# IamJasonBian/Splendor-RL-Gym

Measured on NVIDIA B200. Metric: expanded states/sec (gen+dedup+score+top-k), higher is better.
Workload: dtype u64 keys / f64 scores

## Files before the change

### splendor-rl-gym_b200/csrc/spl_m2.cuh

```cuda
#pragma once
#include "spl_kernels.cuh"

namespace spl {

constexpr int GEM_STATES = 2898;
constexpr int NODE_BM_WORDS = 46;
constexpr int NODE_WORDS = 48;
constexpr uint64_t NODE_OCC = 1ull << 63;
constexpr int SMALL_ITEMS = 32;
constexpr int SMALL_W = 128;
constexpr int SM_TBL = 256;
constexpr int SM_STAGE = 48;
struct GroupArgs;
constexpr int NUM_CLS = 8;
constexpr int CLS_WARP = 6, CLS_CTA = 7;
constexpr int M2_WARPS = TILE / 32;
constexpr int BIG_DONE = 16;
constexpr int BIG_AT_BITS = 24;

__device__ __host__ __forceinline__ void mask_words(uint64_t lo, uint64_t hi, uint64_t &m0, uint64_t &m1) {
    m0 = (lo >> 15) | (hi << 49);
    m1 = (hi & HI_KEY_MASK) >> 15;
}
__device__ __host__ __forceinline__ uint64_t mask_hash(uint64_t m0, uint64_t m1) { return hash_key(m0, m1); }
// ... 181 lines not shown
#pragma unroll
    for (int q = 0; q < SORT_ITEMS; ++q) {
        const int64_t i = wbase + q * 32 + lane;
        const bool ok = i < n;
        v[q] = ok ? v_in[i] : 0;
        const uint32_t d = (uint32_t)(v[q] >> shift) & (SORT_BINS - 1);
        const unsigned act = __ballot_sync(0xffffffffu, ok);
        off[q] = 0;
        if (ok) {
            const unsigned peers = __match_any_sync(act, d);
            const int leader = __ffs(peers) - 1;
            uint32_t old = 0;
            if ((int)lane == leader) {
                old = whist[w][d];
                whist[w][d] = old + __popc(peers);
            }
            old = __shfl_sync(peers, old, leader);
            off[q] = (uint16_t)(old + __popc(peers & ((1u << lane) - 1)));
        }
        __syncwarp();
    }
    __syncthreads();
    {
        const uint32_t d = threadIdx.x;
        uint32_t run = 0;
        for (int ww = 0; ww < TILE / 32; ++ww) {
            const uint32_t c = whist[ww][d];
            whist[ww][d] = run;
            run += c;
        }
        uint32_t tot;
        const uint32_t ex = block_excl_scan(run, warp_sums, tot);
        dbase[d] = ex;
        gbase[d] = matrix_scanned[(uint64_t)d * ntiles + blockIdx.x];
        for (int ww = 0; ww < TILE / 32; ++ww) whist[ww][d] += ex;
    }
    __syncthreads();
#pragma unroll
    for (int q = 0; q < SORT_ITEMS; ++q) {
        const int64_t i = wbase + q * 32 + lane;
        if (i < n) stage[whist[w][(uint32_t)(v[q] >> shift) & (SORT_BINS - 1)] + off[q]] = v[q];
    }
    __syncthreads();
    const uint32_t cnt = (uint32_t)min((int64_t)SORT_TILE, n - tbase);
    for (uint32_t i = threadIdx.x; i < cnt; i += TILE) {
        const uint64_t x = stage[i];
        const uint32_t d = (uint32_t)(x >> shift) & (SORT_BINS - 1);
        v_out[gbase[d] + (i - dbase[d])] = x;
    }
}

constexpr int ITEM_KEY_LO = 34;
constexpr int OS_BITS = 10, OS_BINS = 1 << OS_BITS, OS_MAX_PASSES = 7;
constexpr int OS_DPT = OS_BINS / TILE;
static_assert(OS_DPT == 4, "the one-sweep pass moves the four digits of a thread as one 16-byte word");
constexpr int64_t OS_MAX_ITEMS = 1ll << 30;

__global__ void __launch_bounds__(TILE) os_hist_kernel(const uint64_t *__restrict__ v, int64_t n, int lo_bit, int passes,
                                                       uint32_t *__restrict__ hist) {
    extern __shared__ uint32_t os_sh[];
    for (int i = threadIdx.x; i < passes * OS_BINS; i += TILE) os_sh[i] = 0;
    __syncthreads();
    for (int64_t i = (int64_t)blockIdx.x * TILE + threadIdx.x; i < n; i += (int64_t)gridDim.x * TILE) {
        const uint64_t x = v[i] >> lo_bit;
        for (int p = 0; p < passes; ++p) atomicAdd(&os_sh[p * OS_BINS + ((uint32_t)(x >> (p * OS_BITS)) & (OS_BINS - 1))], 1u);
    }
    __syncthreads();
    for (int i = threadIdx.x; i < passes * OS_BINS; i += TILE) {
        const uint32_t c = os_sh[i];
        if (c) atomicAdd(hist + i, c);
    }
}
__global__ void __launch_bounds__(OS_BINS) os_base_kernel(uint32_t *hist) {
    __shared__ uint32_t ws[OS_BINS / 32];
    uint32_t *h = hist + blockIdx.x * OS_BINS;
    const unsigned lane = threadIdx.x & 31, w = threadIdx.x >> 5;
    const uint32_t c = h[threadIdx.x];
    const uint32_t inc = warp_incl_scan(c);
    if (lane == 31) ws[w] = inc;
    __syncthreads();
    if (w == 0) {
        const uint32_t x = ws[lane], xi = warp_incl_scan(x);
        ws[lane] = xi - x;
    }
    __syncthreads();
    h[threadIdx.x] = inc - c + ws[w];
}

struct OsSmem {
    uint64_t stage[SORT_TILE];
    uint32_t gbase[OS_BINS];
    uint16_t whist[TILE / 32][OS_BINS];
    uint16_t dbase[OS_BINS];
    uint32_t warp_sums[TILE / 32 + 1];
    uint32_t tile;
    uint32_t stage_p[SORT_TILE];
};
template <bool PAIR>
__global__ void __launch_bounds__(TILE, PAIR ? 3 : 4) os_scatter_kernel(const uint64_t *__restrict__ v_in, const uint32_t *__restrict__ p_in,
                                                                        int64_t n, int shift, const uint32_t *__restrict__ base ,
                                                                        uint32_t *status, Counters *ctr, int ticket_id,
                                                                        uint64_t *__restrict__ v_out, uint32_t *__restrict__ p_out) {
    extern __shared__ __align__(16) unsigned char smem_raw[];
    OsSmem &S = *reinterpret_cast<OsSmem *>(smem_raw);
    const unsigned lane = threadIdx.x & 31, w = threadIdx.x >> 5;
    if (threadIdx.x == 0) S.tile = atomicAdd(&ctr->ticket[ticket_id], 1u);
    for (int i = threadIdx.x; i < (TILE / 32) * OS_BINS / 2; i += TILE) reinterpret_cast<uint32_t *>(&S.whist[0][0])[i] = 0;
    __syncthreads();
    const uint32_t tile = S.tile;
    const int64_t tbase = (int64_t)tile * SORT_TILE, wbase = tbase + (int64_t)w * (32 * SORT_ITEMS);
    uint64_t v[SORT_ITEMS];
    uint32_t pl[PAIR ? SORT_ITEMS : 1];
    uint16_t off[SORT_ITEMS];
#pragma unroll
    for (int q = 0; q < SORT_ITEMS; ++q) {
        const int64_t i = wbase + q * 32 + lane;
        v[q] = i < n ? v_in[i] : 0;
        if (PAIR) pl[q] = i < n ? p_in[i] : 0;
    }
#pragma unroll
    for (int q = 0; q < SORT_ITEMS; ++q) {
        const bool ok = wbase + q * 32 + lane < n;
        const uint32_t d = (uint32_t)(v[q] >> shift) & (OS_BINS - 1);
        const unsigned act = __ballot_sync(0xffffffffu, ok);
        off[q] = 0;
        if (ok) {
            const unsigned peers = __match_any_sync(act, d);
            const int leader = __ffs(peers) - 1;
            uint32_t old = 0;
            if ((int)lane == leader) {
                old = S.whist[w][d];
                S.whist[w][d] = (uint16_t)(old + __popc(peers));
            }
            old = __shfl_sync(peers, old, leader);
            off[q] = (uint16_t)(old + __popc(peers & ((1u << lane) - 1)));
        }
        __syncwarp();
    }
    __syncthreads();
    const uint32_t d0 = threadIdx.x * OS_DPT;
    uint32_t cnt[OS_DPT] = {0, 0, 0, 0};
    for (int ww = 0; ww < TILE / 32; ++ww) {
        uint2 x = *reinterpret_cast<uint2 *>(&S.whist[ww][d0]);
        const uint32_t c0 = x.x & 0xffffu, c1 = x.x >> 16, c2 = x.y & 0xffffu, c3 = x.y >> 16;
        x.x = cnt[0] | (cnt[1] << 16); x.y = cnt[2] | (cnt[3] << 16);
        *reinterpret_cast<uint2 *>(&S.whist[ww][d0]) = x;
        cnt[0] += c0; cnt[1] += c1; cnt[2] += c2; cnt[3] += c3;
    }
    constexpr uint32_t VAL = (1u << 30) - 1;
    uint32_t *mine = status + (uint64_t)tile * OS_BINS + d0;
    {
        const uint32_t f = tile == 0 ? 2u << 30 : 1u << 30;
        uint4 a{f | cnt[0], f | cnt[1], f | cnt[2], f | cnt[3]};
        asm volatile("st.volatile.global.v4.u32 [%0], {%1, %2, %3, %4};" ::"l"(mine), "r"(a.x), "r"(a.y), "r"(a.z), "r"(a.w) : "memory");
    }
    {
        uint32_t tot;
        const uint32_t ex = block_excl_scan(cnt[0] + cnt[1] + cnt[2] + cnt[3], S.warp_sums, tot);
        const uint32_t e0 = ex, e1 = e0 + cnt[0], e2 = e1 + cnt[1], e3 = e2 + cnt[2];
        *reinterpret_cast<uint2 *>(&S.dbase[d0]) = uint2{e0 | (e1 << 16), e2 | (e3 << 16)};
        for (int ww = 0; ww < TILE / 32; ++ww) {
            uint2 x = *reinterpret_cast<uint2 *>(&S.whist[ww][d0]);
            x.x += e0 | (e1 << 16); x.y += e2 | (e3 << 16);
            *reinterpret_cast<uint2 *>(&S.whist[ww][d0]) = x;
        }
    }
    __syncthreads();
#pragma unroll
    for (int q = 0; q < SORT_ITEMS; ++q) {
        if (wbase + q * 32 + lane < n) {
            const uint32_t at = S.whist[w][(uint32_t)(v[q] >> shift) & (OS_BINS - 1)] + off[q];
            S.stage[at] = v[q];
            if (PAIR) S.stage_p[at] = pl[q];
        }
    }
    uint32_t ex[OS_DPT] = {0, 0, 0, 0};
    if (tile > 0) {
        unsigned open = 15;
        for (int64_t p = (int64_t)tile - 1; open; --p) {
            const uint32_t *src = status + (uint64_t)p * OS_BINS + d0;
            uint32_t s[OS_DPT];
            bool ready;
            do {
                asm volatile("ld.volatile.global.v4.u32 {%0, %1, %2, %3}, [%4];" : "=r"(s[0]), "=r"(s[1]), "=r"(s[2]), "=r"(s[3]) : "l"(src) : "memory");
                ready = true;
#pragma unroll
                for (int k = 0; k < OS_DPT; ++k) ready = ready && (!((open >> k) & 1) || (s[k] >> 30) != 0);
            } while (!ready);
#pragma unroll
            for (int k = 0; k < OS_DPT; ++k)
                if ((open >> k) & 1) {
                    ex[k] += s[k] & VAL;
                    if ((s[k] >> 30) == 2) open &= ~(1u << k);
                }
        }
        const uint32_t f = 2u << 30;
        asm volatile("st.volatile.global.v4.u32 [%0], {%1, %2, %3, %4};" ::"l"(mine), "r"(f | (ex[0] + cnt[0])), "r"(f | (ex[1] + cnt[1])),
                     "r"(f | (ex[2] + cnt[2])), "r"(f | (ex[3] + cnt[3])) : "memory");
    }
    {
        const uint4 b = *reinterpret_cast<const uint4 *>(base + d0);
        *reinterpret_cast<uint4 *>(&S.gbase[d0]) = uint4{b.x + ex[0], b.y + ex[1], b.z + ex[2], b.w + ex[3]};
    }
    __syncthreads();
    const uint32_t cnt_tile = (uint32_t)min((int64_t)SORT_TILE, n - tbase);
    for (uint32_t i = threadIdx.x; i < cnt_tile; i += TILE) {
        const uint64_t x = S.stage[i];
        const uint32_t d = (uint32_t)(x >> shift) & (OS_BINS - 1);
        const uint32_t to = S.gbase[d] + (i - S.dbase[d]);
        v_out[to] = x;
        if (PAIR) p_out[to] = S.stage_p[i];
    }
}

constexpr int RUN_ITEMS = 8;
__global__ void __launch_bounds__(TILE) m2_runs_kernel(const uint64_t *__restrict__ iv, int64_t n_items, uint32_t np,
                                                       const uint8_t *__restrict__ ntk8,
                                                       uint32_t *__restrict__ run_start, uint32_t *__restrict__ run_wpre,
                                                       uint64_t *status_f, uint64_t *status_w, Counters *ctr, int ticket_id) {
    __shared__ uint32_t warp_sums[TILE / 32 + 1];
    __shared__ uint32_t s_tile;
    __shared__ uint64_t s_fbase, s_wbase;
    if (threadIdx.x == 0) s_tile = atomicAdd(&ctr->ticket[ticket_id], 1u);
    __syncthreads();
    const uint32_t tile = s_tile;
    const int64_t b0 = ((int64_t)tile * TILE + threadIdx.x) * RUN_ITEMS;
    uint32_t flags = 0, w[RUN_ITEMS], fsum = 0, wsum = 0;
    uint64_t prev = (b0 > 0 && b0 - 1 < n_items) ? iv[b0 - 1] >> ITEM_KEY_LO : 0;
#pragma unroll
    for (int q = 0; q < RUN_ITEMS; ++q) {
        const int64_t i = b0 + q;
        w[q] = 0;
        if (i < n_items) {
            const uint64_t v = iv[i], k = v >> ITEM_KEY_LO;
            if (i == 0 || k != prev) { flags |= 1u << q; ++fsum; }
            prev = k;
            const uint32_t id = (uint32_t)v;
            w[q] = id < np ? ntk8[id] : 1u;
            wsum += w[q];
        }
    }
    uint32_t tot;
    const uint32_t ex = block_excl_scan(wsum << 12 | fsum, warp_sums, tot);
    if (threadIdx.x < 32) {
        const uint64_t e = lookback_exclusive(status_f, tile, tot & 0xfffu, 0);
        if (threadIdx.x == 0) s_fbase = e;
    } else if (threadIdx.x < 64) {
        const uint64_t e = lookback_exclusive(status_w, tile, tot >> 12, 0);
        if (threadIdx.x == 32) s_wbase = e;
    }
    __syncthreads();
    uint64_t r = s_fbase + (ex & 0xfffu), wp = s_wbase + (ex >> 12);
#pragma unroll
    for (int q = 0; q < RUN_ITEMS; ++q) {
        if (flags >> q & 1) {
            run_start[r] = (uint32_t)(b0 + q);
            run_wpre[r] = (uint32_t)wp;
            ++r;
        }
        wp += w[q];
    }
    if (b0 <= n_items - 1 && n_items - 1 < b0 + RUN_ITEMS) {
        run_start[r] = (uint32_t)n_items;
        run_wpre[r] = (uint32_t)wp;
// ... 604 lines not shown
```

### splendor-rl-gym_b200/csrc/splendor_b200.cu

```cuda
#include "../../include/splendor_b200.h"

#include <stdarg.h>
#include <stdio.h>
#include <string.h>

#include <algorithm>
#include <string>
#include <vector>

#include "spl_kernels.cuh"
#include "spl_m2.cuh"
#include "spl_shard.cuh"
#include "spl_realistic.cuh"
#include "spl_tables.cuh"

using namespace spl;

static std::string g_create_error;

struct DevBuf {
    void *p = nullptr;
    size_t cap = 0;
    ~DevBuf() { release(); }
    void release() {
// ... 184 lines not shown
            int r_ = fail(nullptr, e2_ == cudaErrorMemoryAllocation ? SPL_E_NOMEM : SPL_E_CUDA, "%s: %s", #call, \
                          cudaGetErrorString(e2_));                                                           \
            delete c;                                                                                         \
            return r_;                                                                                        \
        }                                                                                                     \
    } while (0)
    CKC(cudaSetDevice(c->device));
    size_t free_b = 0, total_b = 0;
    CKC(cudaMemGetInfo(&free_b, &total_b));
    c->max_table_bytes = cfg->max_table_bytes ? cfg->max_table_bytes : (uint64_t)(free_b * 0.6);
    c->chunk_user = cfg->chunk_parents != 0;
    c->chunk_parents = cfg->chunk_parents ? std::min<uint64_t>(cfg->chunk_parents, 16ull << 20) : (4ull << 20);
    c->chunk_parents = std::max<uint64_t>(c->chunk_parents, TILE);
    const HostTables &T = host_tables();
    CKC(cudaMalloc(&c->d_tabs, sizeof(DevTables)));
    CKC(cudaMemcpy(c->d_tabs, &T.dev, sizeof(DevTables), cudaMemcpyHostToDevice));
    CKC(cudaMalloc(&c->d_takes_idx, T.takes_idx.size() * 4));
    CKC(cudaMemcpy(c->d_takes_idx, T.takes_idx.data(), T.takes_idx.size() * 4, cudaMemcpyHostToDevice));
    CKC(cudaMalloc(&c->d_takes_edges, T.takes_edges.size() * 2));
    CKC(cudaMemcpy(c->d_takes_edges, T.takes_edges.data(), T.takes_edges.size() * 2, cudaMemcpyHostToDevice));
    const size_t n_lut = T.lut_pts.size() + T.lut_saved.size() + T.lut_small.size();
    CKC(cudaMalloc(&c->d_lut, n_lut * 8));
    CKC(cudaMemcpy(c->d_lut, T.lut_pts.data(), T.lut_pts.size() * 8, cudaMemcpyHostToDevice));
    CKC(cudaMemcpy(c->d_lut + T.lut_pts.size(), T.lut_saved.data(), T.lut_saved.size() * 8, cudaMemcpyHostToDevice));
    CKC(cudaMemcpy(c->d_lut + T.lut_pts.size() + T.lut_saved.size(), T.lut_small.data(), T.lut_small.size() * 8,
                   cudaMemcpyHostToDevice));
    c->luts.pts = c->d_lut;
    c->luts.saved = c->d_lut + T.lut_pts.size();
    c->luts.small = c->d_lut + T.lut_pts.size() + T.lut_saved.size();
    CKC(cudaMalloc(&c->d_gemrank, T.gemrank.size() * 2));
    CKC(cudaMemcpy(c->d_gemrank, T.gemrank.data(), T.gemrank.size() * 2, cudaMemcpyHostToDevice));
    {
        std::vector<uint16_t> inv(GEM_STATES, 0);
        for (size_t g = 0; g < T.gemrank.size(); ++g)
            if (T.gemrank[g] != 0xFFFF) inv[T.gemrank[g]] = (uint16_t)g;
        CKC(cudaMalloc(&c->d_rankgems, inv.size() * 2));
        CKC(cudaMemcpy(c->d_rankgems, inv.data(), inv.size() * 2, cudaMemcpyHostToDevice));
    }
    CKC(cudaMalloc(&c->d_ctr, sizeof(Counters)));
    CKC(cudaMallocHost(&c->h_ctr, sizeof(Counters)));
    CKC(cudaMalloc(&c->d_sel, sizeof(SelState)));
    CKC(cudaMallocHost(&c->h_sel, sizeof(SelState)));
    CKC(cudaMalloc(&c->d_hist, SEL_BINS * 4));
    CKC(cudaMemset(c->d_hist, 0, SEL_BINS * 4));
    CKC(cudaMalloc(&c->d_dict, sizeof(ScoreDict)));
    for (auto &ev : c->ev) CKC(cudaEventCreate(&ev));
    CKC(cudaFuncSetAttribute(expand_kernel<MODE_PROBE, IDENT_KEY>, cudaFuncAttributeMaxDynamicSharedMemorySize, (int)sizeof(ExpandSmem2)));
    CKC(cudaFuncSetAttribute(expand_kernel<MODE_PROBE, IDENT_PYHASH>, cudaFuncAttributeMaxDynamicSharedMemorySize, (int)sizeof(ExpandSmem2)));
    CKC(cudaFuncSetAttribute(expand_kernel<MODE_LIST, IDENT_KEY>, cudaFuncAttributeMaxDynamicSharedMemorySize, (int)sizeof(ExpandSmem2)));
    CKC(cudaFuncSetAttribute(m2_buys_kernel, cudaFuncAttributeMaxDynamicSharedMemorySize, (int)sizeof(BuySmem)));
    CKC(cudaFuncSetAttribute(m2_group_warp_kernel<false>, cudaFuncAttributeMaxDynamicSharedMemorySize, (int)offsetof(WarpSmem, bsort)));
    CKC(cudaFuncSetAttribute(m2_group_warp_kernel<true>, cudaFuncAttributeMaxDynamicSharedMemorySize, (int)sizeof(WarpSmem)));
    CKC(cudaFuncSetAttribute(m2_group_big_kernel, cudaFuncAttributeMaxDynamicSharedMemorySize, (int)sizeof(BigSmem)));
    CKC(cudaFuncSetAttribute(os_scatter_kernel<false>, cudaFuncAttributeMaxDynamicSharedMemorySize, (int)offsetof(OsSmem, stage_p)));
    CKC(cudaFuncSetAttribute(os_scatter_kernel<true>, cudaFuncAttributeMaxDynamicSharedMemorySize, (int)sizeof(OsSmem)));
    CKC(cudaFuncSetAttribute(gs_buys_route_kernel, cudaFuncAttributeMaxDynamicSharedMemorySize, (int)sizeof(RouteSmem)));
    CKC(cudaMalloc(&c->d_dict2, sizeof(ScoreDict)));
    CKC(cudaMalloc(&c->d_dest, 3 * MAX_RANKS * 8));
    {
        c->max_node_bytes = cfg->max_node_bytes ? cfg->max_node_bytes : (uint64_t)(free_b * 0.5);
        uint64_t nn = cfg->node_slots ? cfg->node_slots : (1ull << 12);
        nn = std::max<uint64_t>(std::min<uint64_t>(nn, c->max_node_bytes / (NODE_WORDS * 8)), 64);
        CKC(cudaMalloc(&c->nodes, nn * NODE_WORDS * 8));
        CKC(cudaMemset(c->nodes, 0, nn * NODE_WORDS * 8));
        c->nn = nn;
    }
    c->rslots_hint = cfg->table_slots;
    uint64_t slots = cfg->table_slots ? cfg->table_slots : (1ull << 22);
    slots = std::min<uint64_t>(slots, c->max_table_bytes / 64 * BUCKET_SLOTS);
    slots = std::max<uint64_t>(slots, 1024);
    if (alloc_table(c, slots, 0) != SPL_OK) {
        g_create_error = c->err;
        delete c;
        return SPL_E_NOMEM;
    }
    CKC(cudaDeviceSynchronize());
#undef CKC
    *out = c;
    return SPL_OK;
}

int32_t spl_destroy(spl_ctx *c) {
    if (!c) return SPL_OK;
    cudaSetDevice(c->device);
    cudaDeviceSynchronize();
    cudaFree(c->table); cudaFree(c->d_tabs); cudaFree(c->d_takes_idx); cudaFree(c->d_takes_edges);
    cudaFree(c->d_lut); cudaFree(c->d_ctr); cudaFreeHost(c->h_ctr); cudaFree(c->d_sel); cudaFreeHost(c->h_sel);
    cudaFree(c->rtable); cudaFree(c->d_hist); cudaFree(c->d_dict); cudaFree(c->d_dict2); cudaFree(c->d_dest); cudaFree(c->nodes); cudaFree(c->d_gemrank); cudaFree(c->d_rankgems);
    for (auto *b : c->pool_links) delete b;
    for (auto &ev : c->ev) if (ev) cudaEventDestroy(ev);
    delete c;
    return SPL_OK;
}

static int reset_visited(spl_ctx *c, cudaStream_t st) {
    CK(c, enter_device(c));
    CK(c, cudaMemsetAsync(c->table, 0, c->nb * 64, st));
    if (c->node_occ) CK(c, cudaMemsetAsync(c->nodes, 0, c->nn * NODE_WORDS * 8, st));
    c->occupied = 0;
    c->node_occ = 0;
    c->epoch = 0;
    return SPL_OK;
}

int32_t spl_reset_visited(spl_ctx *c, void *stream) {
    if (!c) return SPL_E_INVALID;
    NO_LIVE_SOLVER(c, "spl_reset_visited");
// ... 915 lines not shown
    bool grouped = false;
    spl_rconfig rcfg{};
    bool pending = false;
    int64_t pend_n = 0, pend_uniq = 0;
    spl_level_info pend_info{};
    int64_t beam = 300000;
    int64_t n_front = 0;
    int level = 0;
    bool ended = false;
    int64_t goal_rank = -1;
    explicit spl_solver(spl_ctx *ctx) : SolverBufs(ctx) {}
};

static int ensure_nodes(spl_ctx *c, uint64_t need, cudaStream_t st) {
    while ((double)(c->node_occ + need) > 0.6 * (double)c->nn) {
        uint64_t nnn = c->nn * 2;
        if (nnn * NODE_WORDS * 8 > c->max_node_bytes) nnn = c->max_node_bytes / (NODE_WORDS * 8);
        if (nnn <= c->nn + c->nn / 8) break;
        uint64_t *nt = nullptr;
        cudaError_t e = cudaMalloc(&nt, nnn * NODE_WORDS * 8);
        if (e != cudaSuccess) { cudaGetLastError(); break; }
        CK(c, cudaMemsetAsync(nt, 0, nnn * NODE_WORDS * 8, st));
        m2_rehash_kernel<<<nblk((int64_t)c->nn * 32), TILE, 0, st>>>(c->nodes, c->nn, nt, nnn, c->d_ctr);
        ++c->launches;
        CK(c, cudaGetLastError());
        unsigned int err = 0;
        CK(c, cudaMemcpyAsync(&err, &c->d_ctr->error, 4, cudaMemcpyDeviceToHost, st));
        CK(c, cudaStreamSynchronize(st));
        if (err) { cudaFree(nt); return fail(c, SPL_E_TABLE_FULL, "node rehash into %llu slots overflowed a probe sequence", (unsigned long long)nnn); }
        cudaFree(c->nodes);
        c->nodes = nt;
        c->nn = nnn;
    }
    if (c->node_occ + need > c->nn - c->nn / 16)
        return fail(c, SPL_E_TABLE_FULL, "card-set table full: %llu nodes + %llu new vs %llu slots (max_node_bytes=%llu)",
                    (unsigned long long)c->node_occ, (unsigned long long)need, (unsigned long long)c->nn,
                    (unsigned long long)c->max_node_bytes);
    return SPL_OK;
}

static int add_grouped_root(spl_ctx *c, uint64_t lo, uint64_t hi, cudaStream_t st) {
    m2_root_kernel<<<1, 1, 0, st>>>(c->nodes, c->nn, lo, hi, c->d_gemrank, c->d_ctr);
    ++c->launches;
    CK(c, cudaGetLastError());
    c->node_occ = 1;
    c->occupied = 1;
    return SPL_OK;
}

static int onesweep_sort(spl_ctx *c, uint64_t *const k[2], uint32_t *const pl[2], int64_t n, int lo_bit, int nbits, int *cur, cudaStream_t st) {
    const int passes = (nbits + OS_BITS - 1) / OS_BITS;
    if (n <= 1 || passes <= 0) return SPL_OK;
    if (passes > OS_MAX_PASSES || n >= OS_MAX_ITEMS) return fail(c, SPL_E_INVALID, "internal: one-sweep sort of %lld values, %d bits", (long long)n, nbits);
    const unsigned snt = nblk(n, SORT_TILE);
    const size_t status_bytes = (size_t)snt * OS_BINS * 4;
    CK(c, c->os_hist.ensure(OS_MAX_PASSES * OS_BINS * 4, 0, st));
    CK(c, c->os_status.ensure(status_bytes, 0, st));
    CK(c, cudaMemsetAsync(c->os_hist.p, 0, (size_t)passes * OS_BINS * 4, st));
    os_hist_kernel<<<std::min<unsigned>(148 * 8, nblk(n)), TILE, (size_t)passes * OS_BINS * 4, st>>>(k[*cur], n, lo_bit, passes, c->os_hist.as<uint32_t>());
    os_base_kernel<<<passes, OS_BINS, 0, st>>>(c->os_hist.as<uint32_t>());
    c->launches += 2;
    for (int p = 0; p < passes; ++p) {
        CK(c, cudaMemsetAsync(c->os_status.p, 0, status_bytes, st));
        CKS(c, reset_ticket(c, 2, st));
        if (pl)
            os_scatter_kernel<true><<<snt, TILE, sizeof(OsSmem), st>>>(k[*cur], pl[*cur], n, lo_bit + p * OS_BITS, c->os_hist.as<uint32_t>() + p * OS_BINS,
                                                                       c->os_status.as<uint32_t>(), c->d_ctr, 2, k[*cur ^ 1], pl[*cur ^ 1]);
        else
            os_scatter_kernel<false><<<snt, TILE, offsetof(OsSmem, stage_p), st>>>(k[*cur], nullptr, n, lo_bit + p * OS_BITS,
                                                                                   c->os_hist.as<uint32_t>() + p * OS_BINS,
                                                                                   c->os_status.as<uint32_t>(), c->d_ctr, 2, k[*cur ^ 1], nullptr);
        ++c->launches;
        CK(c, cudaGetLastError());
        *cur ^= 1;
    }
    return SPL_OK;
}

static int sort_items(spl_ctx *c, int64_t n_items, int *cur, cudaStream_t st) {
    const unsigned snt = nblk(n_items, SORT_TILE);
    if (n_items < OS_MAX_ITEMS) {
        uint64_t *const k[2] = {c->y[0].as<uint64_t>(), c->y[1].as<uint64_t>()};
        return onesweep_sort(c, k, nullptr, n_items, ITEM_KEY_LO, 64 - ITEM_KEY_LO, cur, st);
    }
    const int lo_bit = ITEM_KEY_LO;
    const size_t msz = (size_t)SORT_BINS * snt;
    CK(c, c->matrix.ensure(msz * 4, 0, st));
    CK(c, c->matrix2.ensure(msz * 4, 0, st));
    const unsigned st_tiles = nblk((int64_t)msz, TILE * SCAN_ITEMS);
    if (n_items > 1)
        for (int shift = lo_bit; shift < 64; shift += SORT_BITS) {
            sort_hist_kernel<<<snt, TILE, 0, st>>>(c->y[*cur].as<uint64_t>(), n_items, shift, c->matrix.as<uint32_t>(), snt);
            CKS(c, prep_status(c, 1, st_tiles, st));
            CKS(c, reset_ticket(c, 2, st));
            scan_u32_kernel<<<st_tiles, TILE, 0, st>>>(c->matrix.as<uint32_t>(), c->matrix2.as<uint32_t>(), (int64_t)msz,
                                                        c->status[1].as<uint64_t>(), c->d_ctr, 2);
            psort_scatter_kernel<<<snt, TILE, 0, st>>>(c->y[*cur].as<uint64_t>(), n_items, shift, c->matrix2.as<uint32_t>(), snt,
                                                        c->y[*cur ^ 1].as<uint64_t>());
            c->launches += 3;
            CK(c, cudaGetLastError());
            *cur ^= 1;
        }
    return SPL_OK;
}

struct GroupRound {
    const Rec *front = nullptr;
    const Rec *brec = nullptr;
    int64_t np = 0, n_items = 0;
    uint64_t n_cands = 0;
    int64_t rank_base = 0;
    const uint64_t *grank = nullptr;
    bool unordered = false;
    DevBuf *out = nullptr;
    int64_t out_base = 0;
    int heuristic = 0, noise = 0, level = 0;
};
struct RoundTimes { float sort, prep, thread, warp, cta; };

static int group_round(spl_ctx *c, const GroupRound &R, int64_t *n_new_out, RoundTimes *t, cudaStream_t st) {
    CK(c, cudaEventRecord(c->ev[1], st));
    int cur = 0;
    CKS(c, sort_items(c, R.n_items, &cur, st));
    const unsigned rt = nblk(R.n_items, TILE * RUN_ITEMS);
    CK(c, c->run_start.ensure((size_t)R.n_items * 4 + 8, 0, st));
    CK(c, c->run_wpre.ensure((size_t)R.n_items * 4 + 8, 0, st));
    CKS(c, prep_status(c, 1, rt, st));
    CKS(c, prep_status(c, 2, rt, st));
    CKS(c, reset_ticket(c, 1, st));
    m2_runs_kernel<<<rt, TILE, 0, st>>>(c->y[cur].as<uint64_t>(), R.n_items, (uint32_t)R.np, c->ntk8.as<uint8_t>(), c->run_start.as<uint32_t>(),
                                         c->run_wpre.as<uint32_t>(), c->status[1].as<uint64_t>(), c->status[2].as<uint64_t>(), c->d_ctr, 1);
    ++c->launches;
    CK(c, cudaGetLastError());
    CK(c, cudaEventRecord(c->ev[2], st));
    CKS(c, read_ctr(c, st));
    const uint64_t n_runs = c->h_ctr->n_runs;
    CKS(c, ensure_nodes(c, n_runs + n_runs / 8 + 64, st));
    CK(c, c->cls_list.ensure((size_t)n_runs * 8 + 16, 0, st));
    const size_t n_out = (size_t)R.out_base + (size_t)R.n_cands;
    CK(c, R.out->ensure(n_out * 32, (size_t)R.out_base * 32, st));
    CK(c, c->sk.ensure(n_out * 8, (size_t)R.out_base * 8, st));
    GroupArgs A;
    A.front = R.front; A.brec = R.brec; A.iv = c->y[cur].as<uint64_t>();
    A.run_start = c->run_start.as<uint32_t>(); A.run_wpre = c->run_wpre.as<uint32_t>();
    A.np = (uint32_t)R.np; A.rank_base = R.rank_base; A.grank = R.grank; A.unordered = R.unordered;
    A.warp_max = R.unordered ? std::min<uint32_t>(BIG_W, BSORT_MAX) : BIG_W;
    A.tabs = c->d_tabs; A.takes_idx = c->d_takes_idx; A.takes_edges = c->d_takes_edges; A.gemrank = c->d_gemrank; A.rankgems = c->d_rankgems;
    A.nodes = c->nodes; A.nn = c->nn; A.out = R.out->as<Rec>(); A.out_sk = c->sk.as<uint64_t>(); A.out_base = (uint64_t)R.out_base;
    for (int k = 0; k < NUM_CLS; ++k) A.cls_list[k] = nullptr;
    A.cls_list[CLS_WARP] = c->cls_list.as<uint32_t>();
    A.cls_list[CLS_CTA] = c->cls_list.as<uint32_t>() + n_runs;
    A.h = R.heuristic; A.noise_mode = R.noise; A.L = c->luts; A.ctr = c->d_ctr;
    CK(c, cudaEventRecord(c->ev[3], st));
    if (R.unordered) m2_group_tiny_kernel<true><<<nblk((int64_t)n_runs), TILE, 0, st>>>(A, (uint32_t)n_runs);
    else m2_group_tiny_kernel<false><<<nblk((int64_t)n_runs), TILE, 0, st>>>(A, (uint32_t)n_runs);
    CK(c, cudaEventRecord(c->ev[4], st));
    CKS(c, reset_ticket(c, 2, st));
    if (R.unordered) m2_group_warp_kernel<true><<<148 * SPL_WARP_CTAS, TILE, sizeof(WarpSmem), st>>>(A);
    else m2_group_warp_kernel<false><<<148 * SPL_WARP_CTAS, TILE, offsetof(WarpSmem, bsort), st>>>(A);
    CK(c, cudaEventRecord(c->ev[5], st));
    m2_group_big_kernel<<<148 * 5, TILE, sizeof(BigSmem), st>>>(A);
    c->launches += 3;
    CK(c, cudaGetLastError());
    CK(c, cudaEventRecord(c->ev[6], st));
    CKS(c, read_ctr(c, st));
    const Counters &h = *c->h_ctr;
    cudaEventElapsedTime(&t->sort, c->ev[1], c->ev[2]);
    cudaEventElapsedTime(&t->prep, c->ev[2], c->ev[3]);
    cudaEventElapsedTime(&t->thread, c->ev[3], c->ev[4]);
    cudaEventElapsedTime(&t->warp, c->ev[4], c->ev[5]);
    cudaEventElapsedTime(&t->cta, c->ev[5], c->ev[6]);
    if (getenv("SPL_DEBUG"))
        fprintf(stderr, "[grouped] L%d np=%lld items=%lld runs=%llu cls=%u/%u/%u new_nodes=%u winners=%llu | sort+runs %.2f prep %.2f thread %.2f warp %.2f cta %.2f ms | nodes %llu/%llu\n",
                R.level, (long long)R.np, (long long)R.n_items, (unsigned long long)n_runs,
                (unsigned)(n_runs - h.n_cls[CLS_WARP] - h.n_cls[CLS_CTA]), h.n_cls[CLS_WARP], h.n_cls[CLS_CTA], h.n_new_nodes,
                (unsigned long long)h.n_emitted, t->sort, t->prep, t->thread, t->warp, t->cta, (unsigned long long)c->node_occ,
                (unsigned long long)c->nn);
    if (h.error == 3)
        return fail(c, SPL_E_CUDA, "level %d: more than %d card sets share one 30-bit sort key in a run of the warp kernel (or more than %d in one of the CTA kernel)",
                    R.level, MAX_SETS, BIG_DONE);
    if (h.error)
        return fail(c, SPL_E_TABLE_FULL, "card-set table full during level %d (device error %u; %llu slots, max_node_bytes=%llu)", R.level,
                    h.error, (unsigned long long)c->nn, (unsigned long long)c->max_node_bytes);
    c->node_occ += h.n_new_nodes;
    c->occupied += h.n_emitted;
    *n_new_out = (int64_t)h.n_emitted;
    return SPL_OK;
}

static int grouped_expand(spl_solver *s, const Rec *front, int64_t n, int64_t *n_uniq_out, int64_t *n_slots_out, int64_t *generated_out,
                          uint64_t *sk_min_out, uint64_t *sk_max_out, float ms[6], cudaStream_t st) {
    spl_ctx *c = s->c;
    const int64_t chunk = c->chunk_user ? (int64_t)c->chunk_parents : (16ll << 20);
    int64_t n_uniq = 0, n_slots = 0, generated = 0;
    uint64_t sk_min = ~0ull, sk_max = 0;
    for (int64_t p0 = 0; p0 < n; p0 += chunk) {
        const int64_t np = std::min<int64_t>(chunk, n - p0);
        const unsigned nt = nblk(np);
        CKS(c, zero_ctr(c, st));
        CK(c, cudaEventRecord(c->ev[0], st));
        CK(c, c->boff2.ensure((size_t)np * 4 + 4, 0, st));
        CK(c, c->ntk8.ensure((size_t)np + 8, 0, st));
        CK(c, c->y[0].ensure((size_t)np * 8 + 8, 0, st));
        CKS(c, prep_status(c, 0, nt, st));
        m2_count_kernel<<<nt, TILE, 0, st>>>(front + p0, np, c->d_tabs, c->d_takes_idx, c->boff2.as<uint32_t>(),
                                              c->y[0].as<uint64_t>(), c->ntk8.as<uint8_t>(), c->status[0].as<uint64_t>(), c->d_ctr, 0);
        ++c->launches;
        CK(c, cudaGetLastError());
        CKS(c, read_ctr(c, st));
        const uint64_t n_takes = c->h_ctr->total_cands, n_buys = c->h_ctr->n_buys, total = n_takes + n_buys;
        generated += (int64_t)total;
        if (total == 0) continue;
        const int64_t n_items = np + (int64_t)n_buys;
        if (total >= 0xFFFFFFFFull || (uint64_t)n_items >= 0xFFFFFFFFull)
            return fail(c, SPL_E_INVALID, "round produced %llu candidates (>= 2^32): lower spl_config.chunk_parents", (unsigned long long)total);
        CK(c, c->y[0].ensure((size_t)n_items * 8 + 8, (size_t)np * 8, st));
        CK(c, c->y[1].ensure((size_t)n_items * 8 + 8, 0, st));
        CK(c, c->brec.ensure((size_t)n_buys * 32 + 32, 0, st));
        if (n_buys) {
            m2_buys_kernel<<<nt, TILE, sizeof(BuySmem), st>>>(front + p0, np, c->d_tabs, c->d_takes_idx, c->boff2.as<uint32_t>(), p0,
                                                               c->brec.as<Rec>(), c->y[0].as<uint64_t>());
            ++c->launches;
            CK(c, cudaGetLastError());
        }
        GroupRound R;
        R.front = front + p0; R.brec = c->brec.as<Rec>(); R.np = np; R.n_items = n_items; R.n_cands = total; R.rank_base = p0;
        R.out = &s->uniq; R.out_base = n_slots; R.heuristic = s->heuristic; R.noise = s->noise; R.level = s->level;
        int64_t n_new = 0;
        RoundTimes t;
        CKS(c, group_round(c, R, &n_new, &t, st));
        if (n_new) { sk_min = std::min<uint64_t>(sk_min, c->h_ctr->sk_min); sk_max = std::max<uint64_t>(sk_max, c->h_ctr->sk_max); }
        n_uniq += n_new;
        n_slots += n_new;
        float t_count;
        cudaEventElapsedTime(&t_count, c->ev[0], c->ev[1]);
        ms[0] += t_count;
        ms[2] += t.sort;
        ms[1] += t.thread + t.warp + t.cta;
        ms[5] += t.warp;
    }
    *n_uniq_out = n_uniq;
    *n_slots_out = n_slots;
    *generated_out = generated;
    *sk_min_out = sk_min;
    *sk_max_out = sk_max;
    return SPL_OK;
}

struct spl_gsolver : SolverBufs {
    int rank = 0, world = 1, goal = 15, heuristic = 0, noise = 0;
    int64_t beam = 0;
    int64_t n_local = 0, n_global = 1;
    int level = 0;
    int64_t r_p0 = 0, r_np = 0;
    uint64_t r_takes = 0, r_buys = 0;
    int64_t counts[MAX_RANKS]{};
    int64_t n_uniq = 0, generated = 0;
    float ms[4] = {0, 0, 0, 0};
    int lt = 0, cut_cur = 0;
    int64_t kept_local = 0;
    explicit spl_gsolver(spl_ctx *ctx) : SolverBufs(ctx) {}
};

extern "C" {

int32_t spl_gs_create(spl_ctx *c, int32_t rank, int32_t world, const spl_key *root_key, uint64_t root_aux, int32_t goal,
                      int32_t heuristic, int64_t beam, int32_t noise, int32_t keep_links, spl_gsolver **out) {
    if (!c || !root_key || !out || world < 1 || world > MAX_RANKS || rank < 0 || rank >= world || beam < 1)
        return fail(c, SPL_E_INVALID, "spl_gs_create: bad arguments (1 <= world <= %d)", MAX_RANKS);
    if (noise != SPL_NOISE_CONST && noise != SPL_NOISE_HASH) return fail(c, SPL_E_INVALID, "spl_gs_create: noise must be const or hash");
    NO_LIVE_SOLVER(c, "spl_gs_create");
    CK(c, enter_device(c));
    cudaStream_t st = 0;
    CKS(c, reset_visited(c, st));
    spl_gsolver *s = new spl_gsolver(c);
    s->rank = rank; s->world = world; s->goal = goal; s->heuristic = heuristic; s->beam = beam; s->noise = noise;
    s->keep_links = keep_links;
    uint64_t m0, m1;
    mask_words(root_key->lo, root_key->hi & HI_KEY_MASK, m0, m1);
    int rc = SPL_OK;
    if ((int)owner_of_mask(m0, m1, (uint32_t)world) == rank) {
        Rec r{root_key->lo, root_key->hi & HI_KEY_MASK, root_aux, ~0ull};
        uint64_t zero = 0;
        cudaError_t e = s->front.ensure(32, 0, st);
        if (e == cudaSuccess) e = s->grank.ensure(8, 0, st);
        if (e == cudaSuccess) e = cudaMemcpyAsync(s->front.p, &r, 32, cudaMemcpyHostToDevice, st);
        if (e == cudaSuccess) e = cudaMemcpyAsync(s->grank.p, &zero, 8, cudaMemcpyHostToDevice, st);
        if (e == cudaSuccess) e = cudaStreamSynchronize(st);
        c->h2d_bytes += 40;
        if (e != cudaSuccess) rc = fail(c, SPL_E_CUDA, "root upload: %s", cudaGetErrorString(e));
// ... 145 lines not shown
    if (e != cudaSuccess) { cudaFree(p); cudaGetLastError(); return fail(c, SPL_E_CUDA, "cudaIpcGetMemHandle: %s", cudaGetErrorString(e)); }
    memcpy(handle_out, &h, 64);
    *ptr_out = p;
    return SPL_OK;
}
int32_t spl_ipc_open(spl_ctx *c, const uint8_t handle[64], void **ptr_out) {
    if (!c || !handle || !ptr_out) return SPL_E_INVALID;
    CK(c, enter_device(c));
    cudaIpcMemHandle_t h;
    memcpy(&h, handle, 64);
    cudaError_t e = cudaIpcOpenMemHandle(ptr_out, h, cudaIpcMemLazyEnablePeerAccess);
    if (e != cudaSuccess) { cudaGetLastError(); return fail(c, SPL_E_CUDA, "cudaIpcOpenMemHandle: %s", cudaGetErrorString(e)); }
    return SPL_OK;
}
int32_t spl_ipc_close(spl_ctx *c, void *ptr) {
    if (!c || !ptr) return SPL_E_INVALID;
    CK(c, enter_device(c));
    CK(c, cudaIpcCloseMemHandle(ptr));
    return SPL_OK;
}
int32_t spl_ipc_free(spl_ctx *c, void *ptr) {
    if (!c || !ptr) return SPL_E_INVALID;
    CK(c, enter_device(c));
    CK(c, cudaDeviceSynchronize());
    CK(c, cudaFree(ptr));
    return SPL_OK;
}

int32_t spl_gs_round_group(spl_gsolver *s, const void *recv_dev, int64_t n_recv, int64_t *n_new_host, void *stream) {
    if (!s || !n_new_host || n_recv < 0) return SPL_E_INVALID;
    spl_ctx *c = s->c;
    cudaStream_t st = (cudaStream_t)stream;
    CK(c, enter_device(c));
    *n_new_host = 0;
    const int64_t np = s->r_np, n_items = np + n_recv;
    const uint64_t total = s->r_takes + (uint64_t)n_recv;
    if (total == 0) return SPL_OK;
    if (total >= 0xFFFFFFFFull || (uint64_t)n_items >= 0xFFFFFFFFull)
        return fail(c, SPL_E_INVALID, "round holds %llu candidates (>= 2^32): use smaller rank windows", (unsigned long long)total);
    CK(c, c->y[0].ensure((size_t)n_items * 8 + 8, (size_t)np * 8, st));
    CK(c, c->y[1].ensure((size_t)n_items * 8 + 8, 0, st));
    CKS(c, zero_ctr(c, st));
    if (n_recv) {
        gs_recv_items_kernel<<<nblk(n_recv), TILE, 0, st>>>(reinterpret_cast<const Rec *>(recv_dev), n_recv, (uint32_t)np, c->y[0].as<uint64_t>());
        ++c->launches;
    }
    GroupRound R;
    R.front = s->front.as<Rec>() + s->r_p0; R.brec = reinterpret_cast<const Rec *>(recv_dev); R.np = np; R.n_items = n_items;
    R.n_cands = total; R.grank = s->grank.as<uint64_t>() + s->r_p0; R.unordered = true; R.out = &s->uniq; R.out_base = s->n_uniq;
    R.heuristic = s->heuristic; R.noise = s->noise; R.level = s->level;
    int64_t n_new = 0;
    RoundTimes t;
    CKS(c, group_round(c, R, &n_new, &t, st));
    s->ms[0] += t.sort + t.prep; s->ms[1] += t.thread; s->ms[2] += t.warp; s->ms[3] += t.cta;
    s->n_uniq += n_new;
    *n_new_host = n_new;
    return SPL_OK;
}

int32_t spl_gs_stage_ms(spl_gsolver *s, float ms_host[4]) {
    if (!s || !ms_host) return SPL_E_INVALID;
    for (int i = 0; i < 4; ++i) ms_host[i] = s->ms[i];
    return SPL_OK;
}

int32_t spl_gs_counters(spl_gsolver *s, int64_t *n_uniq_host, int64_t *generated_host, int64_t *visited_host) {
    if (!s) return SPL_E_INVALID;
    if (n_uniq_host) *n_uniq_host = s->n_uniq;
    if (generated_host) *generated_host = s->generated;
    if (visited_host) *visited_host = (int64_t)s->c->occupied;
    return SPL_OK;
}

int32_t spl_gs_dict(spl_gsolver *s, void **dict_dev, int64_t *bytes, void *stream) {
    if (!s || !dict_dev || !bytes) return SPL_E_INVALID;
    spl_ctx *c = s->c;
    cudaStream_t st = (cudaStream_t)stream;
    CK(c, enter_device(c));
    CK(c, cudaMemsetAsync(c->d_dict->key, 0xFF, sizeof(c->d_dict->key), st));
    CK(c, cudaMemsetAsync(c->d_dict->cnt, 0, sizeof(ScoreDict) - sizeof(c->d_dict->key), st));
    if (s->n_uniq) {
        dict_build_kernel<<<std::min<unsigned>(nblk(s->n_uniq), 148 * 8), TILE, 0, st>>>(c->sk.as<uint64_t>(), s->n_uniq, c->d_dict);
        ++c->launches;
        CK(c, cudaGetLastError());
    }
    *dict_dev = c->d_dict;
    *bytes = (int64_t)sizeof(ScoreDict);
    return SPL_OK;
}

int32_t spl_gs_threshold(spl_gsolver *s, const void *dicts_dev, int64_t k, int64_t n_uniq_global, int32_t *need_ties_host,
                         void *stream) {
    if (!s || !dicts_dev || !need_ties_host || k < 1) return SPL_E_INVALID;
    spl_ctx *c = s->c;
    cudaStream_t st = (cudaStream_t)stream;
    CK(c, enter_device(c));
    CK(c, cudaMemsetAsync(c->d_dict2->key, 0xFF, sizeof(c->d_dict2->key), st));
    CK(c, cudaMemsetAsync(c->d_dict2->cnt, 0, sizeof(ScoreDict) - sizeof(c->d_dict2->key), st));
    memset(c->h_sel, 0, sizeof(SelState));
    c->h_sel->rank_t = ~0ull;
    CK(c, cudaMemcpyAsync(c->d_sel, c->h_sel, sizeof(SelState), cudaMemcpyHostToDevice, st));
    gs_dict_merge_kernel<<<nblk((int64_t)s->world * DICT_CAP), TILE, 0, st>>>(reinterpret_cast<const ScoreDict *>(dicts_dev), s->world, c->d_dict2);
    dict_rank_kernel<<<1, 1024, 0, st>>>(c->d_dict2, (uint64_t)std::min(k, n_uniq_global), 0, c->d_sel);
    c->launches += 2;
    CK(c, cudaGetLastError());
    CK(c, cudaMemcpyAsync(c->h_sel, c->d_sel, sizeof(SelState), cudaMemcpyDeviceToHost, st));
    CK(c, cudaStreamSynchronize(st));
// ... 793 lines not shown
```

Before: 675.8 million.

## Widen one-sweep radix scatter tiles and batch decoupled lookback reads

The one-sweep scatter kernel now runs 512 threads with 16 items each, so tiles are larger and there are fewer tiles and fewer lookback chains. Per-thread digit work drops from four to two. Offsets are packed two per 32-bit register, and the payload staging array is overlaid on the per-warp histogram so shared memory stays bounded. Lookback now reads four predecessor tiles per iteration instead of spinning on one. Payload loads are deferred until after key staging. Sort and run-detection timings are also split into separate events. The larger tiles may lower occupancy.

```diff
diff --git a/splendor-rl-gym_b200/csrc/spl_m2.cuh b/splendor-rl-gym_b200/csrc/spl_m2.cuh
--- a/splendor-rl-gym_b200/csrc/spl_m2.cuh
+++ b/splendor-rl-gym_b200/csrc/spl_m2.cuh
@@ -257,8 +257,11 @@
 
 constexpr int ITEM_KEY_LO = 34;
 constexpr int OS_BITS = 10, OS_BINS = 1 << OS_BITS, OS_MAX_PASSES = 7;
-constexpr int OS_DPT = OS_BINS / TILE;
-static_assert(OS_DPT == 4, "the one-sweep pass moves the four digits of a thread as one 16-byte word");
+constexpr int OS_NT = 512, OS_IPT = 16, OS_TILE = OS_NT * OS_IPT, OS_WARPS = OS_NT / 32;
+constexpr int OS_DPT = OS_BINS / OS_NT;
+constexpr int OS_LOOKBACK = 4;
+static_assert(OS_DPT == 2, "the one-sweep pass moves the two digits of a thread as one 8-byte word");
+static_assert(OS_TILE <= 1 << 15, "tile-local positions are 16-bit and two of them are added as one 32-bit word");
 constexpr int64_t OS_MAX_ITEMS = 1ll << 30;
 
 __global__ void __launch_bounds__(TILE) os_hist_kernel(const uint64_t *__restrict__ v, int64_t n, int lo_bit, int passes,
@@ -293,42 +296,56 @@
 }
 
 struct OsSmem {
-    uint64_t stage[SORT_TILE];
+    uint64_t stage[OS_TILE];
+    union {
+        uint16_t whist[OS_WARPS][OS_BINS];
+        uint32_t stage_p[OS_TILE];
+    };
     uint32_t gbase[OS_BINS];
-    uint16_t whist[TILE / 32][OS_BINS];
     uint16_t dbase[OS_BINS];
-    uint32_t warp_sums[TILE / 32 + 1];
+    uint32_t warp_sums[OS_WARPS];
     uint32_t tile;
-    uint32_t stage_p[SORT_TILE];
 };
+static_assert(sizeof(uint16_t) * OS_WARPS * OS_BINS == sizeof(uint32_t) * OS_TILE, "stage_p exactly overlays whist");
+
+__device__ __forceinline__ uint32_t os_block_excl_scan(uint32_t v, uint32_t *warp_sums ) {
+    const unsigned lane = threadIdx.x & 31, w = threadIdx.x >> 5;
+    const uint32_t inc = warp_incl_scan(v);
+    if (lane == 31) warp_sums[w] = inc;
+    __syncthreads();
+    if (w == 0) {
+        const uint32_t s = lane < OS_WARPS ? warp_sums[lane] : 0, si = warp_incl_scan(s);
+        if (lane < OS_WARPS) warp_sums[lane] = si - s;
+    }
+    __syncthreads();
+    return inc - v + warp_sums[w];
+}
+
 template <bool PAIR>
-__global__ void __launch_bounds__(TILE, PAIR ? 3 : 4) os_scatter_kernel(const uint64_t *__restrict__ v_in, const uint32_t *__restrict__ p_in,
-                                                                        int64_t n, int shift, const uint32_t *__restrict__ base ,
-                                                                        uint32_t *status, Counters *ctr, int ticket_id,
-                                                                        uint64_t *__restrict__ v_out, uint32_t *__restrict__ p_out) {
+__global__ void __launch_bounds__(OS_NT, 2) os_scatter_kernel(const uint64_t *__restrict__ v_in, const uint32_t *__restrict__ p_in,
+                                                              int64_t n, int shift, const uint32_t *__restrict__ base ,
+                                                              uint32_t *status, Counters *ctr, int ticket_id,
+                                                              uint64_t *__restrict__ v_out, uint32_t *__restrict__ p_out) {
     extern __shared__ __align__(16) unsigned char smem_raw[];
     OsSmem &S = *reinterpret_cast<OsSmem *>(smem_raw);
     const unsigned lane = threadIdx.x & 31, w = threadIdx.x >> 5;
     if (threadIdx.x == 0) S.tile = atomicAdd(&ctr->ticket[ticket_id], 1u);
-    for (int i = threadIdx.x; i < (TILE / 32) * OS_BINS / 2; i += TILE) reinterpret_cast<uint32_t *>(&S.whist[0][0])[i] = 0;
+    for (int i = threadIdx.x; i < OS_WARPS * OS_BINS / 2; i += OS_NT) reinterpret_cast<uint32_t *>(&S.whist[0][0])[i] = 0;
     __syncthreads();
     const uint32_t tile = S.tile;
-    const int64_t tbase = (int64_t)tile * SORT_TILE, wbase = tbase + (int64_t)w * (32 * SORT_ITEMS);
-    uint64_t v[SORT_ITEMS];
-    uint32_t pl[PAIR ? SORT_ITEMS : 1];
-    uint16_t off[SORT_ITEMS];
-#pragma unroll
-    for (int q = 0; q < SORT_ITEMS; ++q) {
-        const int64_t i = wbase + q * 32 + lane;
-        v[q] = i < n ? v_in[i] : 0;
-        if (PAIR) pl[q] = i < n ? p_in[i] : 0;
-    }
-#pragma unroll
-    for (int q = 0; q < SORT_ITEMS; ++q) {
-        const bool ok = wbase + q * 32 + lane < n;
+    const int64_t tbase = (int64_t)tile * OS_TILE, wbase = tbase + (int64_t)w * (32 * OS_IPT);
+    const int rem = (int)max((int64_t)-1, min(n - wbase - lane, (int64_t)(32 * OS_IPT)));
+    uint64_t v[OS_IPT];
+    uint32_t at[OS_IPT / 2] = {};
+#pragma unroll
+    for (int q = 0; q < OS_IPT; ++q) {
+        v[q] = q * 32 < rem ? v_in[wbase + q * 32 + lane] : 0;
+    }
+#pragma unroll
+    for (int q = 0; q < OS_IPT; ++q) {
+        const bool ok = q * 32 < rem;
         const uint32_t d = (uint32_t)(v[q] >> shift) & (OS_BINS - 1);
         const unsigned act = __ballot_sync(0xffffffffu, ok);
-        off[q] = 0;
         if (ok) {
             const unsigned peers = __match_any_sync(act, d);
             const int leader = __ffs(peers) - 1;
@@ -338,83 +355,93 @@
                 S.whist[w][d] = (uint16_t)(old + __popc(peers));
             }
             old = __shfl_sync(peers, old, leader);
-            off[q] = (uint16_t)(old + __popc(peers & ((1u << lane) - 1)));
+            at[q / 2] |= (old + __popc(peers & ((1u << lane) - 1))) << (16 * (q & 1));
         }
         __syncwarp();
     }
     __syncthreads();
     const uint32_t d0 = threadIdx.x * OS_DPT;
-    uint32_t cnt[OS_DPT] = {0, 0, 0, 0};
-    for (int ww = 0; ww < TILE / 32; ++ww) {
-        uint2 x = *reinterpret_cast<uint2 *>(&S.whist[ww][d0]);
-        const uint32_t c0 = x.x & 0xffffu, c1 = x.x >> 16, c2 = x.y & 0xffffu, c3 = x.y >> 16;
-        x.x = cnt[0] | (cnt[1] << 16); x.y = cnt[2] | (cnt[3] << 16);
-        *reinterpret_cast<uint2 *>(&S.whist[ww][d0]) = x;
-        cnt[0] += c0; cnt[1] += c1; cnt[2] += c2; cnt[3] += c3;
+    uint32_t c0 = 0, c1 = 0;
+#pragma unroll
+    for (int ww = 0; ww < OS_WARPS; ++ww) {
+        uint32_t *h = reinterpret_cast<uint32_t *>(&S.whist[ww][d0]);
+        const uint32_t x = *h;
+        *h = c0 | (c1 << 16);
+        c0 += x & 0xffffu; c1 += x >> 16;
     }
     constexpr uint32_t VAL = (1u << 30) - 1;
     uint32_t *mine = status + (uint64_t)tile * OS_BINS + d0;
     {
         const uint32_t f = tile == 0 ? 2u << 30 : 1u << 30;
-        uint4 a{f | cnt[0], f | cnt[1], f | cnt[2], f | cnt[3]};
-        asm volatile("st.volatile.global.v4.u32 [%0], {%1, %2, %3, %4};" ::"l"(mine), "r"(a.x), "r"(a.y), "r"(a.z), "r"(a.w) : "memory");
+        asm volatile("st.volatile.global.v2.u32 [%0], {%1, %2};" ::"l"(mine), "r"(f | c0), "r"(f | c1) : "memory");
     }
     {
-        uint32_t tot;
-        const uint32_t ex = block_excl_scan(cnt[0] + cnt[1] + cnt[2] + cnt[3], S.warp_sums, tot);
-        const uint32_t e0 = ex, e1 = e0 + cnt[0], e2 = e1 + cnt[1], e3 = e2 + cnt[2];
-        *reinterpret_cast<uint2 *>(&S.dbase[d0]) = uint2{e0 | (e1 << 16), e2 | (e3 << 16)};
-        for (int ww = 0; ww < TILE / 32; ++ww) {
-            uint2 x = *reinterpret_cast<uint2 *>(&S.whist[ww][d0]);
-            x.x += e0 | (e1 << 16); x.y += e2 | (e3 << 16);
-            *reinterpret_cast<uint2 *>(&S.whist[ww][d0]) = x;
-        }
-    }
-    __syncthreads();
-#pragma unroll
-    for (int q = 0; q < SORT_ITEMS; ++q) {
-        if (wbase + q * 32 + lane < n) {
-            const uint32_t at = S.whist[w][(uint32_t)(v[q] >> shift) & (OS_BINS - 1)] + off[q];
-            S.stage[at] = v[q];
-            if (PAIR) S.stage_p[at] = pl[q];
-        }
-    }
-    uint32_t ex[OS_DPT] = {0, 0, 0, 0};
+        const uint32_t e0 = os_block_excl_scan(c0 + c1, S.warp_sums), e = e0 | ((e0 + c0) << 16);
+        *reinterpret_cast<uint32_t *>(&S.dbase[d0]) = e;
+#pragma unroll
+        for (int ww = 0; ww < OS_WARPS; ++ww) *reinterpret_cast<uint32_t *>(&S.whist[ww][d0]) += e;
+    }
+    __syncthreads();
+#pragma unroll
+    for (int q = 0; q < OS_IPT; ++q) {
+        if (q * 32 < rem) {
+            at[q / 2] += (uint32_t)S.whist[w][(uint32_t)(v[q] >> shift) & (OS_BINS - 1)] << (16 * (q & 1));
+            S.stage[(at[q / 2] >> (16 * (q & 1))) & 0xffffu] = v[q];
+        }
+    }
+    uint32_t pl[PAIR ? OS_IPT : 1];
+    if (PAIR) {
+#pragma unroll
+        for (int q = 0; q < OS_IPT; ++q) {
+            pl[q] = q * 32 < rem ? p_in[wbase + q * 32 + lane] : 0;
+        }
+    }
+    uint32_t ex0 = 0, ex1 = 0;
     if (tile > 0) {
-        unsigned open = 15;
-        for (int64_t p = (int64_t)tile - 1; open; --p) {
-            const uint32_t *src = status + (uint64_t)p * OS_BINS + d0;
-            uint32_t s[OS_DPT];
-            bool ready;
-            do {
-                asm volatile("ld.volatile.global.v4.u32 {%0, %1, %2, %3}, [%4];" : "=r"(s[0]), "=r"(s[1]), "=r"(s[2]), "=r"(s[3]) : "l"(src) : "memory");
-                ready = true;
-#pragma unroll
-                for (int k = 0; k < OS_DPT; ++k) ready = ready && (!((open >> k) & 1) || (s[k] >> 30) != 0);
-            } while (!ready);
-#pragma unroll
-            for (int k = 0; k < OS_DPT; ++k)
-                if ((open >> k) & 1) {
-                    ex[k] += s[k] & VAL;
-                    if ((s[k] >> 30) == 2) open &= ~(1u << k);
-                }
+        unsigned open = 3;
+        for (int64_t p = (int64_t)tile - 1; open;) {
+            uint32_t s0[OS_LOOKBACK], s1[OS_LOOKBACK];
+#pragma unroll
+            for (int j = 0; j < OS_LOOKBACK; ++j) {
+                s0[j] = s1[j] = 2u << 30;
+                if (p - j >= 0)
+                    asm volatile("ld.volatile.global.v2.u32 {%0, %1}, [%2];" : "=r"(s0[j]), "=r"(s1[j]) : "l"(status + (uint64_t)(p - j) * OS_BINS + d0) : "memory");
+            }
+            bool stop = false;
+#pragma unroll
+            for (int j = 0; j < OS_LOOKBACK; ++j) {
+                if (stop || ((open & 1) && (s0[j] >> 30) == 0) || ((open & 2) && (s1[j] >> 30) == 0)) { stop = true; continue; }
+                if (open & 1) { ex0 += s0[j] & VAL; if ((s0[j] >> 30) == 2) open &= ~1u; }
+                if (open & 2) { ex1 += s1[j] & VAL; if ((s1[j] >> 30) == 2) open &= ~2u; }
+                --p;
+                stop = open == 0;
+            }
         }
         const uint32_t f = 2u << 30;
-        asm volatile("st.volatile.global.v4.u32 [%0], {%1, %2, %3, %4};" ::"l"(mine), "r"(f | (ex[0] + cnt[0])), "r"(f | (ex[1] + cnt[1])),
-                     "r"(f | (ex[2] + cnt[2])), "r"(f | (ex[3] + cnt[3])) : "memory");
+        asm volatile("st.volatile.global.v2.u32 [%0], {%1, %2};" ::"l"(mine), "r"(f | (ex0 + c0)), "r"(f | (ex1 + c1)) : "memory");
     }
     {
-        const uint4 b = *reinterpret_cast<const uint4 *>(base + d0);
-        *reinterpret_cast<uint4 *>(&S.gbase[d0]) = uint4{b.x + ex[0], b.y + ex[1], b.z + ex[2], b.w + ex[3]};
-    }
-    __syncthreads();
-    const uint32_t cnt_tile = (uint32_t)min((int64_t)SORT_TILE, n - tbase);
-    for (uint32_t i = threadIdx.x; i < cnt_tile; i += TILE) {
-        const uint64_t x = S.stage[i];
-        const uint32_t d = (uint32_t)(x >> shift) & (OS_BINS - 1);
-        const uint32_t to = S.gbase[d] + (i - S.dbase[d]);
-        v_out[to] = x;
-        if (PAIR) p_out[to] = S.stage_p[i];
+        const uint2 b = *reinterpret_cast<const uint2 *>(base + d0);
+        *reinterpret_cast<uint2 *>(&S.gbase[d0]) = uint2{b.x + ex0, b.y + ex1};
+    }
+    __syncthreads();
+    if (PAIR) {
+#pragma unroll
+        for (int q = 0; q < OS_IPT; ++q)
+            if (q * 32 < rem) S.stage_p[(at[q / 2] >> (16 * (q & 1))) & 0xffffu] = pl[q];
+        __syncthreads();
+    }
+    const uint32_t cnt_tile = (uint32_t)min((int64_t)OS_TILE, n - tbase);
+#pragma unroll
+    for (int q = 0; q < OS_IPT; ++q) {
+        const uint32_t i = threadIdx.x + q * OS_NT;
+        if (i < cnt_tile) {
+            const uint64_t x = S.stage[i];
+            const uint32_t d = (uint32_t)(x >> shift) & (OS_BINS - 1);
+            const uint32_t to = S.gbase[d] + (i - S.dbase[d]);
+            v_out[to] = x;
+            if (PAIR) p_out[to] = S.stage_p[i];
+        }
     }
 }
 
diff --git a/splendor-rl-gym_b200/csrc/splendor_b200.cu b/splendor-rl-gym_b200/csrc/splendor_b200.cu
--- a/splendor-rl-gym_b200/csrc/splendor_b200.cu
+++ b/splendor-rl-gym_b200/csrc/splendor_b200.cu
@@ -260,7 +260,7 @@
     CKC(cudaFuncSetAttribute(m2_group_warp_kernel<false>, cudaFuncAttributeMaxDynamicSharedMemorySize, (int)offsetof(WarpSmem, bsort)));
     CKC(cudaFuncSetAttribute(m2_group_warp_kernel<true>, cudaFuncAttributeMaxDynamicSharedMemorySize, (int)sizeof(WarpSmem)));
     CKC(cudaFuncSetAttribute(m2_group_big_kernel, cudaFuncAttributeMaxDynamicSharedMemorySize, (int)sizeof(BigSmem)));
-    CKC(cudaFuncSetAttribute(os_scatter_kernel<false>, cudaFuncAttributeMaxDynamicSharedMemorySize, (int)offsetof(OsSmem, stage_p)));
+    CKC(cudaFuncSetAttribute(os_scatter_kernel<false>, cudaFuncAttributeMaxDynamicSharedMemorySize, (int)sizeof(OsSmem)));
     CKC(cudaFuncSetAttribute(os_scatter_kernel<true>, cudaFuncAttributeMaxDynamicSharedMemorySize, (int)sizeof(OsSmem)));
     CKC(cudaFuncSetAttribute(gs_buys_route_kernel, cudaFuncAttributeMaxDynamicSharedMemorySize, (int)sizeof(RouteSmem)));
     CKC(cudaMalloc(&c->d_dict2, sizeof(ScoreDict)));
@@ -1282,7 +1282,7 @@
     const int passes = (nbits + OS_BITS - 1) / OS_BITS;
     if (n <= 1 || passes <= 0) return SPL_OK;
     if (passes > OS_MAX_PASSES || n >= OS_MAX_ITEMS) return fail(c, SPL_E_INVALID, "internal: one-sweep sort of %lld values, %d bits", (long long)n, nbits);
-    const unsigned snt = nblk(n, SORT_TILE);
+    const unsigned snt = nblk(n, OS_TILE);
     const size_t status_bytes = (size_t)snt * OS_BINS * 4;
     CK(c, c->os_hist.ensure(OS_MAX_PASSES * OS_BINS * 4, 0, st));
     CK(c, c->os_status.ensure(status_bytes, 0, st));
@@ -1294,12 +1294,11 @@
         CK(c, cudaMemsetAsync(c->os_status.p, 0, status_bytes, st));
         CKS(c, reset_ticket(c, 2, st));
         if (pl)
-            os_scatter_kernel<true><<<snt, TILE, sizeof(OsSmem), st>>>(k[*cur], pl[*cur], n, lo_bit + p * OS_BITS, c->os_hist.as<uint32_t>() + p * OS_BINS,
-                                                                       c->os_status.as<uint32_t>(), c->d_ctr, 2, k[*cur ^ 1], pl[*cur ^ 1]);
+            os_scatter_kernel<true><<<snt, OS_NT, sizeof(OsSmem), st>>>(k[*cur], pl[*cur], n, lo_bit + p * OS_BITS, c->os_hist.as<uint32_t>() + p * OS_BINS,
+                                                                        c->os_status.as<uint32_t>(), c->d_ctr, 2, k[*cur ^ 1], pl[*cur ^ 1]);
         else
-            os_scatter_kernel<false><<<snt, TILE, offsetof(OsSmem, stage_p), st>>>(k[*cur], nullptr, n, lo_bit + p * OS_BITS,
-                                                                                   c->os_hist.as<uint32_t>() + p * OS_BINS,
-                                                                                   c->os_status.as<uint32_t>(), c->d_ctr, 2, k[*cur ^ 1], nullptr);
+            os_scatter_kernel<false><<<snt, OS_NT, sizeof(OsSmem), st>>>(k[*cur], nullptr, n, lo_bit + p * OS_BITS, c->os_hist.as<uint32_t>() + p * OS_BINS,
+                                                                         c->os_status.as<uint32_t>(), c->d_ctr, 2, k[*cur ^ 1], nullptr);
         ++c->launches;
         CK(c, cudaGetLastError());
         *cur ^= 1;
@@ -1346,12 +1345,13 @@
     int64_t out_base = 0;
     int heuristic = 0, noise = 0, level = 0;
 };
-struct RoundTimes { float sort, prep, thread, warp, cta; };
+struct RoundTimes { float sort, runs, prep, thread, warp, cta; };
 
 static int group_round(spl_ctx *c, const GroupRound &R, int64_t *n_new_out, RoundTimes *t, cudaStream_t st) {
     CK(c, cudaEventRecord(c->ev[1], st));
     int cur = 0;
     CKS(c, sort_items(c, R.n_items, &cur, st));
+    CK(c, cudaEventRecord(c->ev[7], st));
     const unsigned rt = nblk(R.n_items, TILE * RUN_ITEMS);
     CK(c, c->run_start.ensure((size_t)R.n_items * 4 + 8, 0, st));
     CK(c, c->run_wpre.ensure((size_t)R.n_items * 4 + 8, 0, st));
@@ -1395,16 +1395,17 @@
     CK(c, cudaEventRecord(c->ev[6], st));
     CKS(c, read_ctr(c, st));
     const Counters &h = *c->h_ctr;
-    cudaEventElapsedTime(&t->sort, c->ev[1], c->ev[2]);
+    cudaEventElapsedTime(&t->sort, c->ev[1], c->ev[7]);
+    cudaEventElapsedTime(&t->runs, c->ev[7], c->ev[2]);
     cudaEventElapsedTime(&t->prep, c->ev[2], c->ev[3]);
     cudaEventElapsedTime(&t->thread, c->ev[3], c->ev[4]);
     cudaEventElapsedTime(&t->warp, c->ev[4], c->ev[5]);
     cudaEventElapsedTime(&t->cta, c->ev[5], c->ev[6]);
     if (getenv("SPL_DEBUG"))
-        fprintf(stderr, "[grouped] L%d np=%lld items=%lld runs=%llu cls=%u/%u/%u new_nodes=%u winners=%llu | sort+runs %.2f prep %.2f thread %.2f warp %.2f cta %.2f ms | nodes %llu/%llu\n",
+        fprintf(stderr, "[grouped] L%d np=%lld items=%lld runs=%llu cls=%u/%u/%u new_nodes=%u winners=%llu | sort %.2f runs %.2f prep %.2f thread %.2f warp %.2f cta %.2f ms | nodes %llu/%llu\n",
                 R.level, (long long)R.np, (long long)R.n_items, (unsigned long long)n_runs,
                 (unsigned)(n_runs - h.n_cls[CLS_WARP] - h.n_cls[CLS_CTA]), h.n_cls[CLS_WARP], h.n_cls[CLS_CTA], h.n_new_nodes,
-                (unsigned long long)h.n_emitted, t->sort, t->prep, t->thread, t->warp, t->cta, (unsigned long long)c->node_occ,
+                (unsigned long long)h.n_emitted, t->sort, t->runs, t->prep, t->thread, t->warp, t->cta, (unsigned long long)c->node_occ,
                 (unsigned long long)c->nn);
     if (h.error == 3)
         return fail(c, SPL_E_CUDA, "level %d: more than %d card sets share one 30-bit sort key in a run of the warp kernel (or more than %d in one of the CTA kernel)",
@@ -1465,7 +1466,7 @@
         float t_count;
         cudaEventElapsedTime(&t_count, c->ev[0], c->ev[1]);
         ms[0] += t_count;
-        ms[2] += t.sort;
+        ms[2] += t.sort + t.runs;
         ms[1] += t.thread + t.warp + t.cta;
         ms[5] += t.warp;
     }
@@ -1717,7 +1718,7 @@
     int64_t n_new = 0;
     RoundTimes t;
     CKS(c, group_round(c, R, &n_new, &t, st));
-    s->ms[0] += t.sort + t.prep; s->ms[1] += t.thread; s->ms[2] += t.warp; s->ms[3] += t.cta;
+    s->ms[0] += t.sort + t.runs + t.prep; s->ms[1] += t.thread; s->ms[2] += t.warp; s->ms[3] += t.cta;
     s->n_uniq += n_new;
     *n_new_host = n_new;
     return SPL_OK;
```

Measured after the change: 702.9 million, median of 6. 1.04x the previous value.
